# noway/nzcp-circom

Hardware: AMD Instinct MI355X
Metric: groth16_proofs_per_sec_nzcp_live (higher is better)
Workload: dtype u32x8 (256-bit Montgomery integers); 1 GPU; nzcp_liveTest.circom = NZCPPubIdentity(1, 355, 0, 4, 2, 4, 6), single proof: nVars=825434, nConstraints=830227, nPublic=513, domain=2^20, nCoefs=4236306; parallelism=1gpu

## Files before the change

### nzcp-circom_amd/csrc/ec29.cuh

```cuda
#pragma once
#include "ec.cuh"
#include "fq29.cuh"

namespace g16 {

using G1Affine29 = Affine<Fq29Ops>;
using G2Affine29 = Affine<Fq2x29Ops>;
using G1XYZZ29 = XYZZ<Fq29Ops>;
using G2XYZZ29 = XYZZ<Fq2x29Ops>;

template <class F> G16_HD bool x29_is_inf(const XYZZ<F>& p) { return F::is_literal_zero(p.zz); }
template <class F> G16_HD void x29_set_inf(XYZZ<F>& p) {
  p.x = F::zero(); p.y = F::zero(); p.zz = F::zero(); p.zzz = F::zero();
}
template <class F> G16_HD bool x29_diff_is_zero(const typename F::T& d) {
  if (!F::template maybe_zero<7>(d)) return false;
  return F::is_zero(d);
}

template <class F> G16_HD void x29_dbl_affine(XYZZ<F>& r, const Affine<F>& p) {
  using T = typename F::T;
  const T U = F::add(p.y, p.y);
  const T V = F::sqr(U);
  const T W = F::mul(U, V);
// ... 64 lines not shown
    acc.y = F::template sub<2>(F::mul(R, F::template sub<6>(Qv, X3)), F::mul(acc.y, PPP));
  }
  acc.x = X3;
  acc.zz = F::mul(acc.zz, PP);
  acc.zzz = F::mul(acc.zzz, PPP);
  return suspicious;
}

template <class F> G16_HD void x29_add(XYZZ<F>& acc, const XYZZ<F>& q) {
  using T = typename F::T;
  if (x29_is_inf(q)) return;
  if (x29_is_inf(acc)) { acc = q; return; }
  const T U1 = F::mul(acc.x, q.zz);
  const T U2 = F::mul(q.x, acc.zz);
  const T S1 = F::mul(acc.y, q.zzz);
  const T S2 = F::mul(q.y, acc.zzz);
  const T P = F::template sub<2>(U2, U1);
  const T R = F::template sub<2>(S2, S1);
  if (x29_diff_is_zero<F>(P)) {
    if (F::is_zero(R)) x29_dbl(acc);
    else x29_set_inf(acc);
    return;
  }
  const T PP = F::sqr(P);
  const T PPP = F::mul(P, PP);
  const T Qv = F::mul(U1, PP);
  const T X3 = F::sub_b_2c(F::sqr(R), PPP, Qv);
  acc.y = F::template sub<2>(F::mul(R, F::template sub<6>(Qv, X3)), F::mul(S1, PPP));
  acc.x = X3;
  acc.zz = F::mul(F::mul(acc.zz, q.zz), PP);
  acc.zzz = F::mul(F::mul(acc.zzz, q.zzz), PPP);
}

template <class F> G16_HD void a29_neg(Affine<F>& p) { p.y = F::template neg<2>(p.y); }

struct alignas(16) F29Packed { uint32_t v[8]; };
G16_HD F29Packed f29_pack(const F29& a) {
  F29Packed r;
#pragma unroll
  for (int w = 0; w < 8; w++) {
    const int bit = 32 * w, i = bit / 29, o = bit % 29;
    uint64_t x = a.l[i] >> o;
    int have = 29 - o;
    if (i + 1 < 9) { x |= (uint64_t)a.l[i + 1] << have; have += 29; }
    if (have < 32 && i + 2 < 9) x |= (uint64_t)a.l[i + 2] << have;
    r.v[w] = (uint32_t)x;
  }
  return r;
}
G16_HD F29 f29_unpack(const F29Packed& p) {
  F29 t;
#pragma unroll
  for (int i = 0; i < 9; i++) {
    const int bit = 29 * i, w = bit >> 5, o = bit & 31;
    uint64_t x = p.v[w];
    if (w + 1 < 8) x |= (uint64_t)p.v[w + 1] << 32;
    t.l[i] = (uint32_t)(x >> o) & (i < 8 ? kM29 : 0xffffffffu);
  }
  t.pad_ = 0;
  return t;
}
template <class F> struct PackedAffine;
template <> struct alignas(64) PackedAffine<Fq29Ops> { F29Packed x, y; };
template <> struct alignas(64) PackedAffine<Fq2x29Ops> { F29Packed xa, xb, ya, yb; };
G16_HD void a29_pack(PackedAffine<Fq29Ops>& r, const Affine<Fq29Ops>& p) { r.x = f29_pack(p.x); r.y = f29_pack(p.y); }
G16_HD void a29_unpack(Affine<Fq29Ops>& r, const PackedAffine<Fq29Ops>& p) { r.x = f29_unpack(p.x); r.y = f29_unpack(p.y); }
// ... 18 lines not shown
```

### nzcp-circom_amd/csrc/msm.cuh

```cuda
#pragma once
#include <stdlib.h>

#include <atomic>

#include "ec29.cuh"
#include "internal.h"

namespace g16 {

struct MsmPlan {
  uint32_t nsec, n;
  uint32_t sec_begin[kMsmMaxSections];
  int c, Ws;
  uint32_t W, pf, B, low_bits, bins, rps, rows, ones;
  uint32_t salt_bits;
  uint32_t dup_rows, dup_bits;
  uint32_t wb, wx;
  uint32_t wkb;
};
__host__ __device__ __forceinline__ uint32_t msm_win_off(const MsmPlan& pl, uint32_t j) { return j * pl.wb + (j < pl.wx ? j : pl.wx); }
__host__ __device__ __forceinline__ uint32_t msm_win_bits(const MsmPlan& pl, uint32_t j) { return pl.wb + (j < pl.wx ? 1u : 0u); }

__host__ __device__ __forceinline__ uint32_t msm_dup_hash(const uint32_t x[8], uint32_t bits) {
  uint64_t h = 0x9E3779B97F4A7C15ull;
// ... 15 lines not shown
  uint64_t max_tasks = 0;
  uint32_t task_len = 0;
  uint32_t task_len_min = 0;
  uint32_t* h_stat = nullptr;
  uint32_t seg_len = 0;
  uint32_t seg_len_lat = 0, seg_len_thr = 0;
  uint32_t row_pts = 0;
  uint32_t* d_off = nullptr;
  uint32_t* d_toff = nullptr;
  uint32_t* d_foff = nullptr;
  uint32_t* d_tile_a = nullptr;
  uint32_t* d_tile_b = nullptr;
  uint32_t* d_tile_c = nullptr;
  uint2* d_task_desc = nullptr;
  uint4* d_qdesc = nullptr;
  uint32_t* d_class = nullptr;
  uint32_t* d_queue = nullptr;
  uint32_t* d_redo = nullptr;
  void* d_partial = nullptr;
  void* d_bsum = nullptr;
  uint32_t* d_heavy = nullptr;
  uint32_t* d_medium = nullptr;
  uint32_t max_heavy = 0;
  void* d_seg = nullptr;
  void* d_red = nullptr;
  bool reduce_scan = false;
  void* d_canon = nullptr;
  void* d_dseg = nullptr;
  void* d_dred = nullptr;
  hipStream_t st_dup = nullptr;
  hipEvent_t ev_dup_fork = nullptr, ev_dup_join = nullptr;
  uint32_t* d_dcount = nullptr;
  uint32_t* d_dlist = nullptr;
  uint32_t nsec_lane = 0;
  uint8_t* h_pinned = nullptr;
  bool rows_mapped = false;
  size_t out_bytes = 0;
  hipEvent_t ev0 = nullptr, ev1 = nullptr;
  hipEvent_t ev_done = nullptr;
  hipEvent_t trace_ev[4] = {};
  float last_accum_ms = 0.f;
  hipEvent_t gate = nullptr;
  uint32_t waves_per_simd = 0;
  uint32_t chunk_quota = 0;
};

struct MsmWorkspace {
  uint32_t* d_hist = nullptr;
  uint32_t* d_bin_cnt = nullptr;
  uint32_t* d_bin_start = nullptr;
  uint2* d_tmp = nullptr;
  uint32_t* d_sorted = nullptr;
  uint32_t* d_cnt = nullptr;
  uint32_t nb = 0;
  uint32_t* d_dup_cnt = nullptr;
  uint32_t* d_dup_rep = nullptr;
  uint32_t* d_dup_mixed = nullptr;
  const Fr* d_scalars = nullptr;
  bool direct = false;
  uint32_t bin_cap = 0;
  uint32_t dup_chunk = 16, dup_bit_rows = 16;
  uint32_t* h_over = nullptr;
  hipStream_t st_last = nullptr, st2_last = nullptr;
  MsmLaneWs lane[2];
  hipEvent_t ev_sorted = nullptr;
  hipEvent_t trace_ev[4] = {};
  bool launched = false;
  bool empty = false;
};

struct U256 { uint32_t v[8]; };

inline uint32_t msm_seg_len_cfg(int which) {
  struct Cfg { uint32_t v[3]; };
  static const Cfg cfg = [] {
    Cfg c{{8u, 4u, 8u}};
    if (const char* e = getenv("G16_SEG_LEN")) {
      int a = 0, b = 0, d = 0;
      const int k = sscanf(e, "%d,%d,%d", &a, &b, &d);
      if (k >= 1 && a > 0) c.v[0] = (uint32_t)a;
      if (k >= 2 && b > 0) c.v[1] = (uint32_t)b;
      if (k >= 3 && d > 0) c.v[2] = (uint32_t)d;
    }
    for (auto& x : c.v) x = x > 64 ? 64 : x;
    return c;
  }();
  return cfg.v[which];
}

static constexpr uint32_t kTailThreads = 256;
static constexpr uint32_t kRemClasses = 32;
static constexpr uint32_t kTaskChunk = 64;
static constexpr uint32_t kLightTasks = 3;
static constexpr uint32_t kMediumTasks = 64;

struct MsmSmallInit { uint32_t *h_stat, *d_class, *d_queue, *d_heavy, *d_medium; };
int msm_front_end(const MsmGroup& g, MsmWorkspace* ws, const Fr* d_scalars, hipStream_t st);
int msm_build_queue(const MsmGroup& g, MsmWorkspace* ws, MsmLaneWs& ln, hipStream_t st);
int msm_launch_lane_g2(const MsmGroup& g, MsmWorkspace* ws, MsmLaneWs& ln, hipStream_t st);
int msm_convert_bases_g2(const void* in, void* out, uint32_t n);
int msm_precompute_g2(const void* in, void* out, uint32_t n, int ndbl);

template <class F>
__global__ __launch_bounds__(64, F::kAccumWavesPerSimd) void msm_accumulate_kernel(const PackedAffine<F>* __restrict__ bases,
                                                            const uint32_t* __restrict__ sorted,
                                                            const uint32_t* __restrict__ toff, uint32_t nbk,
                                                            uint32_t point_base,
                                                            const uint4* __restrict__ qdesc,
                                                            uint32_t* __restrict__ queue,
                                                            uint32_t* __restrict__ redo,
                                                            XYZZ<F>* __restrict__ partial, uint32_t chunk_quota) {
  const uint32_t total = toff[nbk];
  uint32_t pulled = 0;
  const uint32_t lane = threadIdx.x;
  const unsigned long long lt_mask = (1ull << lane) - 1;
  constexpr uint32_t kNone = 0xffffffffu;
  uint32_t next = 0, chunk_end = 0;
  bool exhausted = false;
  uint32_t my_task = kNone, pending = kNone, cur = 0, end = 0;
  bool bad = false;
  uint4 desc = make_uint4(0, 0, 0, 0);
  XYZZ<F> acc;
  x29_set_inf(acc);
  for (;;) {
    if (my_task != kNone && cur == end) {
      partial[my_task] = acc;
      if (bad) redo[atomicAdd(&queue[1], 1u)] = my_task;
      my_task = kNone;
    }
// ... 461 lines not shown
      if (k == 0 && live) {
        x29_to_canon<F, typename F::CanonOps>(r, v);
        o[0] = r;
      }
    } else {
      for (int d = (int)kPairGroup >> 1; d >= 1; d >>= 1) x29_tree_step<F, (int)kPairGroup>(y, d, k);
      if (k == 0 && live) {
        x29_to_canon<F, typename F::CanonOps>(r, y);
        o[1] = r;
        x29_to_canon<F, typename F::CanonOps>(r, t);
        o[2] = r;
      }
    }
  }
}

static __global__ __launch_bounds__(256) void msm_dup_compact_kernel(const uint32_t* __restrict__ toff, uint32_t B, uint32_t rps,
                                                              uint32_t dup_row0, uint32_t dup_bits, uint32_t sec0,
                                                              uint32_t nsec_lane, const uint32_t* __restrict__ dup_cnt,
                                                              const uint32_t* __restrict__ dup_mixed,
                                                              uint32_t* __restrict__ dcount, uint32_t* __restrict__ dlist) {
  __builtin_amdgcn_s_setprio(3);
  const uint32_t i = blockIdx.x * blockDim.x + threadIdx.x;
  if (i >= (nsec_lane << dup_bits)) return;
  const uint32_t sl = i >> dup_bits, hb = i & ((1u << dup_bits) - 1);
  const size_t di = ((size_t)(sec0 + sl) << dup_bits) + hb;
  if (dup_cnt[di] < kDupMin || dup_mixed[di]) return;
  const uint32_t key = (sl * rps + dup_row0) * B + hb;
  if (toff[key + 1] == toff[key]) return;
  const uint32_t k = atomicAdd(&dcount[sl], 1u);
  dlist[((size_t)sl << dup_bits) + k] = hb;
}

template <class F>
__global__ __launch_bounds__(kTailThreads) void msm_dup_bits_kernel(const XYZZ<F>* __restrict__ partial,
                                                              const XYZZ<F>* __restrict__ bsum,
                                                              const uint32_t* __restrict__ toff, uint32_t B,
                                                              uint32_t rps, uint32_t dup_row0, uint32_t dup_bits,
                                                              uint32_t sec0, uint32_t nsec_lane, uint32_t nchunk,
                                                              uint32_t chunk_bits, uint32_t bit_rows,
                                                              const uint32_t* __restrict__ dcount,
                                                              const uint32_t* __restrict__ dlist,
                                                              const uint32_t* __restrict__ dup_rep,
                                                              const Fr* __restrict__ scalars,
                                                              const uint32_t* __restrict__ src,
                                                              XYZZ<F>* __restrict__ dseg) {
  __builtin_amdgcn_s_setprio(3);
  const uint32_t wid = blockIdx.x * (blockDim.x >> 6) + (threadIdx.x >> 6), lane = threadIdx.x & 63u;
  const uint32_t nrow = nsec_lane * bit_rows;
  if (wid >= nrow * nchunk) return;
  const uint32_t chunk = wid / nrow, row = wid % nrow, bit = row % bit_rows, sl = row / bit_rows;
  const uint32_t wave = row * nchunk + chunk;
  const uint32_t count = dcount[sl], k = chunk * 64 + lane;
  XYZZ<F> acc;
  x29_set_inf(acc);
  if (chunk * 64 < count) {
    if (k < count) {
      const uint32_t hb = dlist[((size_t)sl << dup_bits) + k];
      const Fr v = scalars[src[dup_rep[((size_t)(sec0 + sl) << dup_bits) + hb]]];
      const uint32_t pos = bit * chunk_bits;
      uint64_t w2 = v.v[pos >> 5];
      if ((pos >> 5) + 1 < 8) w2 |= (uint64_t)v.v[(pos >> 5) + 1] << 32;
      const uint32_t cv = (uint32_t)(w2 >> (pos & 31)) & ((1u << chunk_bits) - 1u);
      if (cv) {
        const XYZZ<F> t = msm_bucket_value<F>(partial, bsum, toff, (sl * rps + dup_row0) * B + hb);
        msm_mul_small(acc, t, cv);
      }
    }
    for (int d = 32; d >= 1; d >>= 1) x29_tree_step<F>(acc, d, lane);
  }
  if (lane == 0) dseg[wave] = acc;
}

template <class F>
__global__ __launch_bounds__(kTailThreads) void msm_wave_reduce_kernel(const XYZZ<F>* __restrict__ in, uint32_t nin,
                                                             XYZZ<F>* __restrict__ out, uint32_t nout) {
  __builtin_amdgcn_s_setprio(3);
  const uint32_t j = blockIdx.y, blk = blockIdx.x * (blockDim.x >> 6) + (threadIdx.x >> 6), lane = threadIdx.x & 63u;
  if (blk >= nout) return;
  const uint32_t i = blk * 64 + lane;
  XYZZ<F> p;
  if (i < nin) p = in[(size_t)j * nin + i];
  else x29_set_inf(p);
  for (int d = 32; d >= 1; d >>= 1) x29_tree_step<F>(p, d, lane);
  if (lane == 0) out[(size_t)j * nout + blk] = p;
}

template <class F>
__global__ __launch_bounds__(256) void msm_convert_bases_kernel(const Affine<typename F::CanonOps>* __restrict__ in,
                                                                PackedAffine<F>* __restrict__ out, uint32_t n) {
  const uint32_t i = blockIdx.x * blockDim.x + threadIdx.x;
  if (i >= n) return;
  Affine<F> r;
  a29_from_canon<F, typename F::CanonOps>(r, in[i]);
  PackedAffine<F> pk;
  a29_pack(pk, r);
  out[i] = pk;
}
template <class FC>
__global__ __launch_bounds__(256) void msm_precompute_kernel(const Affine<FC>* __restrict__ in,
                                                             Affine<FC>* __restrict__ out, uint32_t n, int ndbl) {
  const uint32_t i = blockIdx.x * blockDim.x + threadIdx.x;
// ... 115 lines not shown
  uint32_t quota = 0xffffffffu;
  if (ln.chunk_quota) {
    quota = ln.chunk_quota;
    waves = (max_chunks + quota - 1) / quota + 64;
  }
  if (waves > max_chunks) waves = max_chunks;
  if (waves == 0) waves = 1;
  if (ln.gate) G16_HIP(hipStreamWaitEvent(st, ln.gate, 0));
  G16_HIP(hipEventRecord(ln.ev0, st));
  msm_accumulate_kernel<F><<<(unsigned)waves, 64, 0, st>>>((const PackedAffine<F>*)d_bases, ws->d_sorted, ln.d_toff, nbk,
                                                            ln.point_base, ln.d_qdesc, ln.d_queue, ln.d_redo,
                                                            (PT*)ln.d_partial, quota);
  G16_HIP(hipEventRecord(ln.ev1, st));
  msm_redo_kernel<F><<<64, 64, 0, st>>>((const PackedAffine<F>*)d_bases, ws->d_sorted, ln.point_base, ln.d_task_desc,
                                        ln.d_queue, ln.d_redo, (PT*)ln.d_partial);
  msm_combine_light_kernel<FT><<<(nbk + kTailThreads - 1) / kTailThreads, kTailThreads, 0, st>>>((const TPT*)ln.d_partial, ln.d_toff, nbk,
                                                              (TPT*)ln.d_bsum, ln.d_heavy, ln.max_heavy, ln.d_medium,
                                                              msm_light_max(ln), ln.h_stat);
  msm_combine_medium_kernel<FT><<<1024, kTailThreads, 0, st>>>((const TPT*)ln.d_partial, ln.d_toff, (TPT*)ln.d_bsum, ln.d_medium,
                                                              ln.max_heavy);
  msm_combine_heavy_kernel<FT><<<2048, kTailThreads, 0, st>>>((const TPT*)ln.d_partial, ln.d_toff, (TPT*)ln.d_bsum,
                                                   ln.d_heavy, ln.max_heavy);
  mark(1);
  uint32_t nout_pts = ln.row_pts;
  if (g.dup_rows) {
    hipStream_t sd = ln.st_dup ? ln.st_dup : st;
    if (sd != st) {
      G16_HIP(hipEventRecord(ln.ev_dup_fork, st));
      G16_HIP(hipStreamWaitEvent(sd, ln.ev_dup_fork, 0));
    }
    const uint32_t nchunk = (1u << g.dup_bits) >> 6, drows = ln.nsec_lane * ws->dup_bit_rows;
    const uint32_t waves_d = drows * nchunk;
    const uint32_t sec0 = ln.key_lo / (g.rps * g.B), dup_row0 = (uint32_t)g.W + (g.ones ? 1u : 0u);
    G16_HIP(hipMemsetAsync(ln.d_dcount, 0, 16, sd));
    msm_dup_compact_kernel<<<((ln.nsec_lane << g.dup_bits) + 255) / 256, 256, 0, sd>>>(
        ln.d_toff, g.B, g.rps, dup_row0, g.dup_bits, sec0, ln.nsec_lane, ws->d_dup_cnt, ws->d_dup_mixed, ln.d_dcount, ln.d_dlist);
    msm_dup_bits_kernel<FT><<<(waves_d + 3) / 4, kTailThreads, 0, sd>>>(
        (const TPT*)ln.d_partial, (const TPT*)ln.d_bsum, ln.d_toff, g.B, g.rps, dup_row0, g.dup_bits, sec0, ln.nsec_lane, nchunk,
        ws->dup_chunk, ws->dup_bit_rows, ln.d_dcount, ln.d_dlist, ws->d_dup_rep, ws->d_scalars, g.d_src, (TPT*)ln.d_dseg);
    TPT* dcur = (TPT*)ln.d_dseg;
    uint32_t dcnt = nchunk;
    TPT* dbufs[2] = {(TPT*)ln.d_dred, (TPT*)ln.d_dred + (size_t)drows * ((nchunk + 63) / 64)};
    int dflip = 0;
    while (dcnt > 1) {
      const uint32_t nout = (dcnt + 63) / 64;
      msm_wave_reduce_kernel<FT><<<dim3((nout + 3) / 4, drows), kTailThreads, 0, sd>>>(dcur, dcnt, dbufs[dflip], nout);
      dcur = dbufs[dflip];
      dflip ^= 1;
      dcnt = nout;
    }
    msm_to_canon_kernel<F><<<(drows + 63) / 64, 64, 0, sd>>>((const PT*)dcur, (CPT*)ln.d_canon + ln.row_pts, drows);
    G16_HIP(hipGetLastError());
    nout_pts += drows;
    if (sd != st) G16_HIP(hipEventRecord(ln.ev_dup_join, sd));
  }
  if (ln.reduce_scan) {
    const MsmReducePlan rp = msm_reduce_plan(g, ln);
    msm_bucket_reduce_kernel<FT><<<ln.rows * rp.nwg, rp.wg, 0, st>>>((const TPT*)ln.d_partial, (const TPT*)ln.d_bsum, ln.d_toff, rp,
                                                                     (TPT*)ln.d_seg, (CPT*)ln.d_canon);
    mark(2);
    if (rp.nwg > 1) {
      const uint32_t ngroups = (rp.nwg + kPairGroup - 1) / kPairGroup, gpw = 64u / kPairGroup;
      if (ngroups == 1)
        msm_pairs_fold_kernel<FT, true><<<(ln.rows + gpw - 1) / gpw, 64, 0, st>>>((const TPT*)ln.d_seg, rp, 1u, (CPT*)ln.d_canon);
      else
        msm_pairs_fold_kernel<FT, false><<<2 * ((ln.rows * ngroups + gpw - 1) / gpw), 64, 0, st>>>((const TPT*)ln.d_seg, rp, ngroups,
                                                                                            (CPT*)ln.d_canon);
    }
  } else {
    const uint32_t seg_len = ln.seg_len;
    const uint32_t nseg = (g.B + seg_len - 1) / seg_len;
    const uint32_t wave_tree = (nseg % kTailThreads == 0) ? 2u : ((nseg % 64 == 0) ? 1u : 0u);
// ... 32 lines not shown
```

### nzcp-circom_amd/csrc/msm_g1.hip

```cpp
#include <string.h>

#include "msm.cuh"

namespace g16 {

size_t msm_point_bytes(int curve) { return curve == 2 ? sizeof(G2XYZZ) : sizeof(G1XYZZ); }

__device__ __forceinline__ uint32_t msm_extract(const uint32_t s[8], int pos, int c) {
  const int word = pos >> 5, off = pos & 31;
  if (word >= 8) return 0;
  uint64_t v = s[word];
  if (word + 1 < 8) v |= (uint64_t)s[word + 1] << 32;
  return (uint32_t)(v >> off) & ((1u << c) - 1);
}

__device__ __forceinline__ bool msm_load_scalar(const Fr* __restrict__ scalars, const uint32_t* __restrict__ src,
                                                uint32_t g, const U256& K, uint32_t s[8], uint32_t* bits = nullptr) {
  const Fr x = scalars[src ? src[g] : g];
  uint32_t hi = 0;
#pragma unroll
  for (int k = 1; k < 8; k++) hi |= x.v[k];
  const bool one = (hi == 0 && x.v[0] == 1);
  if (bits) {
    uint32_t b = 0;
// ... 349 lines not shown
  __builtin_amdgcn_s_setprio(3);
  __shared__ uint32_t sh_a[256], sh_b[256], sh_c[256];
  const uint32_t tid = threadIdx.x, base = blockIdx.x * kScanTile + tid * 8;
  uint32_t sa = 0, sb = 0, sc = 0;
#pragma unroll
  for (int k = 0; k < 8; k++) {
    const uint32_t v = (base + k < nb) ? cnt[base + k] : 0u;
    sa += v;
    sb += (v + tl - 1) / tl;
    sc += v / tl;
  }
  sh_a[tid] = sa; sh_b[tid] = sb; sh_c[tid] = sc;
  __syncthreads();
  for (uint32_t d = 128; d > 0; d >>= 1) {
    if (tid < d) { sh_a[tid] += sh_a[tid + d]; sh_b[tid] += sh_b[tid + d]; sh_c[tid] += sh_c[tid + d]; }
    __syncthreads();
  }
  if (tid == 0) { tile_a[blockIdx.x] = sh_a[0]; tile_b[blockIdx.x] = sh_b[0]; tile_c[blockIdx.x] = sh_c[0]; }
}

static __global__ __launch_bounds__(1024) void msm_scan_top_kernel(uint32_t* __restrict__ tile_a,
                                                            uint32_t* __restrict__ tile_b,
                                                            uint32_t* __restrict__ tile_c, uint32_t ntiles,
                                                            const uint32_t* __restrict__ off_base,
                                                            uint32_t* __restrict__ total_a,
                                                            uint32_t* __restrict__ total_b,
                                                            uint32_t* __restrict__ total_c, uint32_t max_tasks,
                                                            MsmSmallInit init) {
  __builtin_amdgcn_s_setprio(3);
  __shared__ uint32_t sh_a[1024], sh_b[1024], sh_c[1024];
  const uint32_t tid = threadIdx.x;
  if (tid < 2 * kRemClasses) init.d_class[tid] = 0;
  if (tid < 2) init.d_queue[tid] = 0;
  if (tid == 0) { init.d_heavy[0] = 0; init.d_medium[0] = 0; init.h_stat[3] = 0; }
  const uint32_t chunk = (ntiles + 1023) / 1024;
  const uint32_t lo = tid * chunk, hi = (lo + chunk < ntiles) ? lo + chunk : ntiles;
  uint32_t sa = 0, sb = 0, sc = 0;
  for (uint32_t k = lo; k < hi; k++) { sa += tile_a[k]; sb += tile_b[k]; sc += tile_c[k]; }
  sh_a[tid] = sa; sh_b[tid] = sb; sh_c[tid] = sc;
  __syncthreads();
  for (uint32_t d = 1; d < 1024; d <<= 1) {
    uint32_t va = 0, vb = 0, vc = 0;
    if (tid >= d) { va = sh_a[tid - d]; vb = sh_b[tid - d]; vc = sh_c[tid - d]; }
    __syncthreads();
    sh_a[tid] += va; sh_b[tid] += vb; sh_c[tid] += vc;
    __syncthreads();
  }
  uint32_t pa = sh_a[tid] - sa, pb = sh_b[tid] - sb, pc = sh_c[tid] - sc;
  for (uint32_t k = lo; k < hi; k++) {
    const uint32_t va = tile_a[k], vb = tile_b[k], vc = tile_c[k];
    tile_a[k] = pa; tile_b[k] = pb; tile_c[k] = pc;
    pa += va; pb += vb; pc += vc;
  }
  if (tid == 1023) {
    const uint32_t over = sh_b[1023] > max_tasks ? 1u : 0u;
    init.d_queue[2] = over;
    init.h_stat[2] = over ? sh_b[1023] : 0u;
    *total_a = *off_base + sh_a[1023];
    *total_b = over ? 0u : sh_b[1023];
    *total_c = over ? 0u : sh_c[1023];
    init.h_stat[0] = *off_base + sh_a[1023];
    init.h_stat[1] = *off_base;
  }
}

static __global__ __launch_bounds__(256) void msm_scan_apply_kernel(const uint32_t* __restrict__ cnt, uint32_t nb,
// ... 410 lines not shown
  ln.seg_len_lat = ln.seg_len_thr = ln.seg_len;
  if (ln.reduce_scan && g.dense && !getenv("G16_SEG_LEN")) {
    uint32_t t = ln.seg_len * 2;
    if (g.salt_bits)
      while (t > ln.seg_len && (t > (1u << g.salt_bits) || ((1u << g.salt_bits) % t) != 0)) t >>= 1;
    if (t * 64u <= g.B) ln.seg_len_thr = t;
  }
  const MsmReducePlan rp = msm_reduce_plan(g, ln);
  if (ln.reduce_scan) {
    G16_HIP(hipMalloc(&ln.d_seg, 2 * (size_t)ln.rows * rp.nwg * pb + 256));
  } else {
    const uint64_t nseg = (g.B + ln.seg_len - 1) / ln.seg_len;
    G16_HIP(hipMalloc(&ln.d_seg, (size_t)ln.rows * nseg * pb + 256));
    G16_HIP(hipMalloc(&ln.d_red, 2 * (size_t)ln.rows * ((nseg + 63) / 64) * pb + 256));
  }
  ln.nsec_lane = ln.rows / g.rps;
  ln.row_pts = ln.reduce_scan ? ln.rows * msm_row_out_points(rp) : ln.rows;
  size_t out_pts = ln.row_pts;
  if (g.dup_rows) {
    const size_t nchunk = ((size_t)1 << g.dup_bits) >> 6, drows = (size_t)ln.nsec_lane * g.dup_rows_cap;
    out_pts += drows;
    G16_HIP(hipMalloc(&ln.d_dseg, drows * nchunk * pb + 256));
    G16_HIP(hipMalloc(&ln.d_dred, 2 * drows * ((nchunk + 63) / 64) * pb + 256));
    G16_HIP(hipMalloc(&ln.d_dcount, 64));
    if (curve == 2) {
      int plo = 0, phi = 0;
      G16_HIP(hipDeviceGetStreamPriorityRange(&plo, &phi));
      if (t_aux_prio != kMsmPrioHighest) phi = t_aux_prio;
      G16_HIP(hipStreamCreateWithPriority(&ln.st_dup, hipStreamNonBlocking, phi));
    }
    G16_HIP(hipEventCreateWithFlags(&ln.ev_dup_fork, hipEventDisableTiming));
    G16_HIP(hipEventCreateWithFlags(&ln.ev_dup_join, hipEventDisableTiming));
    G16_HIP(hipMalloc(&ln.d_dlist, ((size_t)ln.nsec_lane << g.dup_bits) * 4 + 64));
  }
  ln.out_bytes = out_pts * cpb;
  G16_HIP(hipHostMalloc((void**)&ln.h_pinned, ln.out_bytes + 256));
  ln.rows_mapped = !(getenv("G16_ROWS_COPY") && atoi(getenv("G16_ROWS_COPY")));
  if (ln.rows_mapped) G16_HIP(hipHostGetDevicePointer(&ln.d_canon, ln.h_pinned, 0));
  else G16_HIP(hipMalloc(&ln.d_canon, ln.out_bytes + 256));
  G16_HIP(hipEventCreate(&ln.ev0));
  G16_HIP(hipEventCreate(&ln.ev1));
  G16_HIP(hipEventCreate(&ln.ev_done));
  return G16_OK;
}

static void lane_destroy(MsmLaneWs& ln) {
  void* ptrs[] = {ln.d_task_desc, ln.d_qdesc, ln.d_class, ln.d_queue, ln.d_redo, ln.d_partial, ln.d_bsum, ln.d_heavy, ln.d_medium,
                  ln.d_seg, ln.d_red, ln.rows_mapped ? nullptr : ln.d_canon, ln.d_off, ln.d_toff, ln.d_foff, ln.d_tile_a, ln.d_tile_b, ln.d_tile_c,
                  ln.d_dseg, ln.d_dred, ln.d_dcount, ln.d_dlist};
  for (void* p : ptrs)
    if (p) (void)hipFree(p);
  if (ln.h_pinned) (void)hipHostFree(ln.h_pinned);
  if (ln.h_stat) (void)hipHostFree(ln.h_stat);
  if (ln.st_dup) (void)hipStreamDestroy(ln.st_dup);
  hipEvent_t evs[] = {ln.ev0, ln.ev1, ln.ev_done, ln.trace_ev[0], ln.trace_ev[1], ln.trace_ev[2], ln.trace_ev[3],
                      ln.ev_dup_fork, ln.ev_dup_join};
  for (hipEvent_t e : evs)
    if (e) (void)hipEventDestroy(e);
  ln = MsmLaneWs();
}

int msm_workspace_create(MsmWorkspace** out, const MsmGroup& g) {
  MsmWorkspace* ws = new MsmWorkspace();
  *out = ws;
  if (g.n == 0) return G16_OK;
  msm_set_throughput(ws, g, false);
  const uint32_t nrb = g.rows * g.bins;
  ws->nb = g.rows * g.B;
  G16_HIP(hipMalloc(&ws->d_hist, ((size_t)g.chunks * nrb + 4) * 4));
  G16_HIP(hipMalloc(&ws->d_bin_cnt, ((size_t)nrb + 4) * 4));
  G16_HIP(hipMalloc(&ws->d_bin_start, ((size_t)nrb + 4) * 4));
  {
    const bool off = getenv("G16_NO_DIRECT_BIN") && atoi(getenv("G16_NO_DIRECT_BIN"));
    uint64_t cap = (g.max_entries * 5 / 2) / nrb + 1024;
    if (const char* e = getenv("G16_TEST_BIN_CAP"))
      if (atoll(e) > 0) cap = (uint64_t)atoll(e);
    ws->direct = g.dense && g.nsec == 1 && !g.ones && !g.dup_rows && !off && cap * nrb < 0x7fffffffull;
    ws->bin_cap = ws->direct ? (uint32_t)cap : 0u;
  }
  G16_HIP(hipHostMalloc((void**)&ws->h_over, 64));
  ws->h_over[0] = 0;
  uint64_t tmp_entries = g.max_entries;
// ... 69 lines not shown
    msm_bin_sort_kernel<<<nrb, 256, 0, st>>>(ws->d_tmp, ws->d_bin_start, pl, ws->d_bin_cnt, ws->bin_cap, ws->h_over, ws->d_cnt,
                                             ws->d_sorted);
    mark(3);
  } else {
    msm_bin_pass_kernel<0><<<g.chunks, kBinThreads, lds, st>>>(d_scalars, g.d_src, pl, K, g.per, g.chunks, ws->d_hist, nullptr,
                                                               ws->d_dup_cnt, ws->d_dup_mixed, nullptr);
    mark(0);
    msm_bin_chunkscan_kernel<<<nrb, 64, 0, st>>>(ws->d_hist, g.chunks, ws->d_bin_cnt);
    msm_bin_scan_kernel<<<1, 1024, 0, st>>>(ws->d_bin_cnt, nrb, ws->d_bin_start, 0xffffffffu);
    mark(1);
    msm_bin_pass_kernel<1><<<g.chunks, kBinThreads, lds, st>>>(d_scalars, g.d_src, pl, K, g.per, g.chunks, ws->d_hist,
                                                               ws->d_bin_start, ws->d_dup_cnt, ws->d_dup_mixed, ws->d_tmp);
    mark(2);
    msm_bin_sort_kernel<<<nrb, 256, 0, st>>>(ws->d_tmp, ws->d_bin_start, pl, nullptr, 0u, nullptr, ws->d_cnt, ws->d_sorted);
    mark(3);
  }
  G16_HIP(hipGetLastError());
  G16_HIP(hipEventRecord(ws->ev_sorted, st));
  return G16_OK;
}

int msm_build_queue(const MsmGroup& g, MsmWorkspace* ws, MsmLaneWs& ln, hipStream_t st) {
  const uint32_t nbk = ln.key_hi - ln.key_lo;
  const uint32_t* cnt = ws->d_cnt + ln.key_lo;
  const uint32_t* off_base = ws->d_bin_start + (size_t)(ln.key_lo / g.B) * g.bins;
  const uint32_t ntiles = (nbk + kScanTile - 1) / kScanTile;
  if (!g.task_len_forced && ln.h_stat[0] > ln.h_stat[1]) {
    const uint64_t e = ln.h_stat[0] - ln.h_stat[1];
    ln.task_len = msm_task_len_for(e / (ln.curve == 2 ? 131072u : 262144u), ln.task_len_min);
  }
  msm_scan_tiles_kernel<<<ntiles, 256, 0, st>>>(cnt, nbk, ln.task_len, ln.d_tile_a, ln.d_tile_b, ln.d_tile_c);
  msm_scan_top_kernel<<<1, 1024, 0, st>>>(ln.d_tile_a, ln.d_tile_b, ln.d_tile_c, ntiles, off_base, ln.d_off + nbk,
                                          ln.d_toff + nbk, ln.d_foff + nbk, (uint32_t)ln.max_tasks,
                                          MsmSmallInit{ln.h_stat, ln.d_class, ln.d_queue, ln.d_heavy, ln.d_medium});
  msm_scan_apply_kernel<<<ntiles, 256, 0, st>>>(cnt, nbk, ln.task_len, ln.d_tile_a, ln.d_tile_b, ln.d_tile_c, off_base,
                                                ln.d_queue, ln.d_off, ln.d_toff, ln.d_foff, ln.d_class);
  msm_task_fill_kernel<<<(nbk + 255) / 256, 256, 0, st>>>(ln.d_off, ln.d_toff, ln.d_foff, nbk, ln.task_len, ln.d_task_desc,
                                                          ln.d_qdesc, ln.d_class, ln.d_class + kRemClasses,
                                                          (uint32_t)ln.max_tasks);
  G16_HIP(hipGetLastError());
  return G16_OK;
}

int msm_launch_front(const MsmGroup& g, MsmWorkspace* ws, const Fr* d_scalars, hipStream_t st) {
  ws->launched = true;
  ws->st_last = st;
  ws->st2_last = nullptr;
  ws->empty = (g.n == 0);
  for (auto& ln : ws->lane) ln.last_accum_ms = 0.f;
  if (g.n == 0) return G16_OK;
  return msm_front_end(g, ws, d_scalars, st);
}

int msm_launch_lanes(const MsmGroup& g, MsmWorkspace* ws, hipStream_t st, hipStream_t st2, hipEvent_t gate1,
                     hipEvent_t gate2) {
  if (g.n == 0) return G16_OK;
  int rc;
  ws->st2_last = st2;
  if (ws->lane[1].active) {
    hipStream_t s2 = st2 ? st2 : st;
    if (s2 != st) G16_HIP(hipStreamWaitEvent(s2, ws->ev_sorted, 0));
    ws->lane[1].gate = gate2;
    if ((rc = msm_launch_lane_g2(g, ws, ws->lane[1], s2))) return rc;
  }
  if (ws->lane[0].active) {
    ws->lane[0].gate = gate1;
    rc = msm_launch_lane_t<Fq29Ops>(g, ws, ws->lane[0], g.d_bases, st);
// ... 10 lines not shown

hipEvent_t msm_event(MsmWorkspace* ws, int which) {
  switch (which) {
    case 0: return ws->ev_sorted;
    case 1: return ws->lane[0].ev0;
    case 2: return ws->lane[0].ev1;
    case 3: return ws->lane[0].active ? ws->lane[0].ev_done : nullptr;
    default: return ws->lane[1].active ? ws->lane[1].ev_done : nullptr;
  }
}

int msm_collect(const MsmGroup& g, MsmWorkspace* ws, MsmResult* out, const std::function<void(const MsmResult&)>* after_g1) {
  for (auto& p : out->g1) xyzz_set_inf(p);
  xyzz_set_inf(out->g2);
  if (!ws->launched || ws->empty) return G16_OK;
  bool overflow = false;
  for (int l = 0; l < 2; l++) {
    MsmLaneWs& ln = ws->lane[l];
    if (!ln.active) continue;
    G16_HIP(hipEventSynchronize(ln.ev_done));
    static const bool trace = getenv("G16_TRACE_HOST") != nullptr;
    if (trace) fprintf(stderr, "[g16 tail] %s lane %d: host saw its row sums at %.3f ms\n", g.dup_rows ? "W" : "H", l, trace_ms());
    (void)hipEventElapsedTime(&ln.last_accum_ms, ln.ev0, ln.ev1);
    if (ln.h_stat[2] || ln.h_stat[3]) {
      set_error(ln.h_stat[2] ? "msm: lane " + std::to_string(l) + " needed " + std::to_string(ln.h_stat[2]) +
                                   " bucket tasks, its buffers hold " + std::to_string(ln.max_tasks)
                             : "msm: lane " + std::to_string(l) + " overflowed its heavy-bucket list");
      overflow = true;
      continue;
    }
    if (g.dup_rows && getenv("G16_DEBUG_DUP")) {
      uint32_t dc[4] = {0, 0, 0, 0};
      (void)hipMemcpy(dc, ln.d_dcount, 16, hipMemcpyDeviceToHost);
      fprintf(stderr, "[g16 dup] lane %d: repeated-value buckets per section: %u %u %u\n", l, dc[0], dc[1], dc[2]);
    }
    const MsmReducePlan rp = msm_reduce_plan(g, ln);
    const uint32_t ngroups = (rp.nwg + kPairGroup - 1) / kPairGroup;
    if (l == 0) {
      const G1XYZZ* rows = reinterpret_cast<const G1XYZZ*>(ln.h_pinned);
      std::vector<G1XYZZ> folded;
      if (ln.reduce_scan && rp.nwg > kPairGroup) {
        folded.resize(ln.rows);
        for (uint32_t r = 0; r < ln.rows; r++)
          msm_fold_row<FqOps>(folded[r], rows + (size_t)r * ngroups * 3, ngroups, rp, msm_row_kind(rp, r));
      }
      const G1XYZZ* rsum = !folded.empty() ? folded.data() : rows;
      const bool merged = g.dup_rows && ws->dup_chunk == (uint32_t)g.c && ws->dup_bit_rows == (uint32_t)g.W;
      std::vector<G1XYZZ> wrow;
      for (int s = 0; s < g.nsec; s++) {
        const G1XYZZ* rs = rsum + (size_t)s * g.rps;
        const G1XYZZ* dup = rows + ln.row_pts + (size_t)s * ws->dup_bit_rows;
        if (merged) {
          wrow.assign(rs, rs + g.W + (g.ones ? 1 : 0));
          for (int j = 0; j < g.W; j++) xyzz_add(wrow[j], dup[j]);
          rs = wrow.data();
        }
        msm_combine_windows<FqOps>(out->g1[s], rs, g.W, g.c, g.ones);
        if (g.dup_rows && !merged) msm_add_bit_sums<FqOps>(out->g1[s], dup, ws->dup_chunk, ws->dup_bit_rows);
      }
      if (after_g1 && *after_g1) (*after_g1)(*out);
    } else {
      const G2XYZZ* rows = reinterpret_cast<const G2XYZZ*>(ln.h_pinned);
      std::vector<G2XYZZ> folded;
      if (ln.reduce_scan && rp.nwg > kPairGroup) {
        folded.resize(ln.rows);
        for (uint32_t r = 0; r < ln.rows; r++)
          msm_fold_row<Fq2Ops>(folded[r], rows + (size_t)r * ngroups * 3, ngroups, rp, msm_row_kind(rp, r));
      }
      const G2XYZZ* rsum = !folded.empty() ? folded.data() : rows;
      const bool merged = g.dup_rows && ws->dup_chunk == (uint32_t)g.c && ws->dup_bit_rows == (uint32_t)g.W;
      std::vector<G2XYZZ> wrow;
      if (merged) {
        wrow.assign(rsum, rsum + g.W + (g.ones ? 1 : 0));
        for (int j = 0; j < g.W; j++) xyzz_add(wrow[j], rows[ln.row_pts + j]);
        rsum = wrow.data();
      }
      msm_combine_windows<Fq2Ops>(out->g2, rsum, g.W, g.c, g.ones);
      if (g.dup_rows && !merged) msm_add_bit_sums<Fq2Ops>(out->g2, rows + ln.row_pts, ws->dup_chunk, ws->dup_bit_rows);
    }
  }
  if (overflow) return G16_E_STATE;
  if (ws->direct && ws->h_over[0]) {
    ws->direct = false;
    ws->h_over[0] = 0;
    int rc = msm_launch_front(g, ws, ws->d_scalars, ws->st_last);
    if (!rc) rc = msm_launch_lanes(g, ws, ws->st_last, ws->st2_last, nullptr, nullptr);
    if (rc) return rc;
    return msm_collect(g, ws, out, after_g1);
  }
  return G16_OK;
}

float msm_last_accum_ms(const MsmWorkspace* ws, int lane) { return ws->lane[lane & 1].last_accum_ms; }
void msm_set_throughput(MsmWorkspace* ws, const MsmGroup& g, bool on) {
  if (!ws) return;
  ws->dup_chunk = on ? g.dup_chunk_wide : g.dup_chunk;
  ws->dup_bit_rows = (254 + ws->dup_chunk - 1) / ws->dup_chunk;
  for (auto& ln : ws->lane)
    if (ln.active) ln.seg_len = on ? ln.seg_len_thr : ln.seg_len_lat;
}
void msm_set_waves(MsmWorkspace* ws, uint32_t waves_g1, uint32_t waves_g2) {
  ws->lane[0].waves_per_simd = waves_g1;
  ws->lane[1].waves_per_simd = waves_g2;
}
void msm_set_quota(MsmWorkspace* ws, uint32_t quota_g1, uint32_t quota_g2) {
  ws->lane[0].chunk_quota = quota_g1;
  ws->lane[1].chunk_quota = quota_g2;
}
float msm_event_offset_ms(MsmWorkspace* ws, hipEvent_t base, int lane, int which) {
  float t = 0.f;
  const MsmLaneWs& ln = ws->lane[lane & 1];
  hipEvent_t e = which < 4 ? ws->trace_ev[which] : which == 4 ? ln.ev0 : which == 5 ? ln.ev1 : ln.trace_ev[(which - 6) & 3];
  if (e && hipEventQuery(e) == hipSuccess) (void)hipEventElapsedTime(&t, base, e);
  return t;
}

}
```

Baseline: 282.6 proofs/s.

## Precompute per-position multiple tables for repeated-value buckets in dup-bit MSM

Adds a table kernel that, for each repeated-value bucket, precomputes multiples 1..15 of the bucket point shifted by each 4-bit sub-position of the chunk. The dup-bits kernel then sums table lookups instead of running a double-and-add scalar multiply for every bit row. This removes redundant small-scalar multiplications repeated across rows, at the cost of a large extra device buffer, an extra launch, and XYZZ table reads. It also folds the dcount memset into the scan-top init kernel, saving one async memset. The table path is enabled only in throughput mode.

```diff
diff --git a/nzcp-circom_amd/csrc/ec29.cuh b/nzcp-circom_amd/csrc/ec29.cuh
--- a/nzcp-circom_amd/csrc/ec29.cuh
+++ b/nzcp-circom_amd/csrc/ec29.cuh
@@ -120,6 +120,55 @@
   acc.zzz = F::mul(F::mul(acc.zzz, q.zzz), PPP);
 }
 
+static constexpr uint32_t kDupSubBits = 4;
+static constexpr uint32_t kDupTabMul = (1u << kDupSubBits) - 1;
+static constexpr uint32_t kDupTabPosMax = 4;
+G16_HD uint32_t x29_dup_positions(uint32_t chunk_bits) { return (chunk_bits + kDupSubBits - 1) / kDupSubBits; }
+G16_HD uint32_t x29_dup_pos_max(uint32_t chunk_bits, uint32_t p) {
+  const uint32_t w = chunk_bits - kDupSubBits * p;
+  return w >= kDupSubBits ? kDupTabMul : (1u << w) - 1u;
+}
+static constexpr uint32_t kDupSplitPos = 3;
+template <class F> G16_HD void x29_dup_table_range(XYZZ<F>* tab, const XYZZ<F>& t, uint32_t p, uint32_t jlo, uint32_t jhi) {
+  const uint32_t nbase = kDupSubBits * p;
+  const uint32_t nd = nbase + (jlo == 1 ? (jhi >= 2 ? 1u : 0u) : 3u);
+  XYZZ<F> cur = t, b = t;
+  for (uint32_t i = 0; i < nd; i++) {
+    x29_dbl(cur);
+    if (i + 1 == nbase) b = cur;
+  }
+  uint32_t j = 9;
+  if (jlo == 1) {
+    tab[0] = b;
+    if (jhi < 2) return;
+    tab[1] = cur;
+    j = 3;
+  }
+  for (; j <= jhi; j++) {
+    x29_add(cur, b);
+    tab[j - 1] = cur;
+  }
+}
+G16_HD bool x29_dup_table_half_range(uint32_t p, uint32_t half, uint32_t jmax, uint32_t& jlo, uint32_t& jhi) {
+  const bool split = p >= kDupSplitPos && jmax > 8u;
+  jlo = half ? 9u : 1u;
+  jhi = (half || !split) ? jmax : 8u;
+  return half == 0 || split;
+}
+template <class F> G16_HD void x29_dup_chunk_entry(XYZZ<F>& q, const XYZZ<F>* tab, uint32_t cv, uint32_t p) {
+  const uint32_t d = (cv >> (kDupSubBits * p)) & kDupTabMul;
+  if (d) q = tab[p * kDupTabMul + d - 1];
+  else x29_set_inf(q);
+}
+template <class F> G16_HD void x29_dup_chunk_sum(XYZZ<F>& acc, const XYZZ<F>* tab, uint32_t cv, uint32_t npos) {
+  x29_set_inf(acc);
+  for (uint32_t p = 0; p < npos; p++) {
+    XYZZ<F> e;
+    x29_dup_chunk_entry(e, tab, cv, p);
+    x29_add(acc, e);
+  }
+}
+
 template <class F> G16_HD void a29_neg(Affine<F>& p) { p.y = F::template neg<2>(p.y); }
 
 struct alignas(16) F29Packed { uint32_t v[8]; };
diff --git a/nzcp-circom_amd/csrc/msm.cuh b/nzcp-circom_amd/csrc/msm.cuh
--- a/nzcp-circom_amd/csrc/msm.cuh
+++ b/nzcp-circom_amd/csrc/msm.cuh
@@ -71,6 +71,8 @@
   hipEvent_t ev_dup_fork = nullptr, ev_dup_join = nullptr;
   uint32_t* d_dcount = nullptr;
   uint32_t* d_dlist = nullptr;
+  void* d_dtab = nullptr;
+  size_t dtab_bytes = 0;
   uint32_t nsec_lane = 0;
   uint8_t* h_pinned = nullptr;
   bool rows_mapped = false;
@@ -99,6 +101,7 @@
   bool direct = false;
   uint32_t bin_cap = 0;
   uint32_t dup_chunk = 16, dup_bit_rows = 16;
+  bool dup_tables = false;
   uint32_t* h_over = nullptr;
   hipStream_t st_last = nullptr, st2_last = nullptr;
   MsmLaneWs lane[2];
@@ -133,7 +136,8 @@
 static constexpr uint32_t kLightTasks = 3;
 static constexpr uint32_t kMediumTasks = 64;
 
-struct MsmSmallInit { uint32_t *h_stat, *d_class, *d_queue, *d_heavy, *d_medium; };
+struct MsmSmallInit { uint32_t *h_stat, *d_class, *d_queue, *d_heavy, *d_medium, *d_dcount; };
+static constexpr uint32_t kDupTabCap = 1024;
 int msm_front_end(const MsmGroup& g, MsmWorkspace* ws, const Fr* d_scalars, hipStream_t st);
 int msm_build_queue(const MsmGroup& g, MsmWorkspace* ws, MsmLaneWs& ln, hipStream_t st);
 int msm_launch_lane_g2(const MsmGroup& g, MsmWorkspace* ws, MsmLaneWs& ln, hipStream_t st);
@@ -661,7 +665,49 @@
   dlist[((size_t)sl << dup_bits) + k] = hb;
 }
 
-template <class F>
+__host__ __device__ __forceinline__ uint32_t msm_dup_chunk_value(const uint32_t v[8], uint32_t row, uint32_t chunk_bits) {
+  const uint32_t pos = row * chunk_bits;
+  uint64_t w2 = v[pos >> 5];
+  if ((pos >> 5) + 1 < 8) w2 |= (uint64_t)v[(pos >> 5) + 1] << 32;
+  return (uint32_t)(w2 >> (pos & 31)) & ((1u << chunk_bits) - 1u);
+}
+
+template <class F>
+__global__ __launch_bounds__(kTailThreads) void msm_dup_table_kernel(const XYZZ<F>* __restrict__ partial,
+                                                               const XYZZ<F>* __restrict__ bsum,
+                                                               const uint32_t* __restrict__ toff, uint32_t B,
+                                                               uint32_t rps, uint32_t dup_row0, uint32_t dup_bits,
+                                                               uint32_t sec0, uint32_t nsec_lane, uint32_t nchunk_tab,
+                                                               uint32_t chunk_bits, uint32_t bit_rows,
+                                                               const uint32_t* __restrict__ dcount,
+                                                               const uint32_t* __restrict__ dlist,
+                                                               const uint32_t* __restrict__ dup_rep,
+                                                               const Fr* __restrict__ scalars,
+                                                               const uint32_t* __restrict__ src,
+                                                               XYZZ<F>* __restrict__ tab) {
+  __builtin_amdgcn_s_setprio(3);
+  const uint32_t wid = blockIdx.x * (blockDim.x >> 6) + (threadIdx.x >> 6), lane = threadIdx.x & 63u;
+  const uint32_t npos = x29_dup_positions(chunk_bits), nrow = nsec_lane * npos * 2u;
+  if (wid >= nrow * nchunk_tab) return;
+  const uint32_t chunk = wid / nrow, r = wid % nrow, half = r & 1u, p = (r >> 1) % npos, sl = (r >> 1) / npos;
+  uint32_t count = dcount[sl];
+  if (count > kDupTabCap) count = kDupTabCap;
+  const uint32_t k = chunk * 64 + lane, jmax = x29_dup_pos_max(chunk_bits, p);
+  uint32_t jlo, jhi;
+  if (k >= count || !x29_dup_table_half_range(p, half, jmax, jlo, jhi)) return;
+  const uint32_t hb = dlist[((size_t)sl << dup_bits) + k];
+  const Fr v = scalars[src[dup_rep[((size_t)(sec0 + sl) << dup_bits) + hb]]];
+  bool need = false;
+  for (uint32_t row = 0; row < bit_rows; row++) {
+    const uint32_t d = (msm_dup_chunk_value(v.v, row, chunk_bits) >> (kDupSubBits * p)) & kDupTabMul;
+    need |= d >= jlo && d <= jhi;
+  }
+  if (!need) return;
+  const XYZZ<F> t = msm_bucket_value<F>(partial, bsum, toff, (sl * rps + dup_row0) * B + hb);
+  x29_dup_table_range(tab + (((size_t)sl * kDupTabCap + k) * npos + p) * kDupTabMul, t, p, jlo, jhi);
+}
+
+template <class F, bool TAB>
 __global__ __launch_bounds__(kTailThreads) void msm_dup_bits_kernel(const XYZZ<F>* __restrict__ partial,
                                                               const XYZZ<F>* __restrict__ bsum,
                                                               const uint32_t* __restrict__ toff, uint32_t B,
@@ -673,6 +719,7 @@
                                                               const uint32_t* __restrict__ dup_rep,
                                                               const Fr* __restrict__ scalars,
                                                               const uint32_t* __restrict__ src,
+                                                              const XYZZ<F>* __restrict__ tab,
                                                               XYZZ<F>* __restrict__ dseg) {
   __builtin_amdgcn_s_setprio(3);
   const uint32_t wid = blockIdx.x * (blockDim.x >> 6) + (threadIdx.x >> 6), lane = threadIdx.x & 63u;
@@ -683,20 +730,46 @@
   const uint32_t count = dcount[sl], k = chunk * 64 + lane;
   XYZZ<F> acc;
   x29_set_inf(acc);
-  if (chunk * 64 < count) {
+  if (!TAB) {
+    if (chunk * 64 < count) {
+      if (k < count) {
+        const uint32_t hb = dlist[((size_t)sl << dup_bits) + k];
+        const Fr v = scalars[src[dup_rep[((size_t)(sec0 + sl) << dup_bits) + hb]]];
+        const uint32_t cv = msm_dup_chunk_value(v.v, bit, chunk_bits);
+        if (cv) {
+          const XYZZ<F> t = msm_bucket_value<F>(partial, bsum, toff, (sl * rps + dup_row0) * B + hb);
+          msm_mul_small(acc, t, cv);
+        }
+      }
+      for (int d = 32; d >= 1; d >>= 1) x29_tree_step<F>(acc, d, lane);
+    }
+  } else if (chunk * 64 < count) {
+    const bool tabbed = chunk * 64 < kDupTabCap;
+    const uint32_t npos = x29_dup_positions(chunk_bits);
+    const XYZZ<F>* mine = tab + ((size_t)sl * kDupTabCap + (tabbed ? k : 0u)) * npos * kDupTabMul;
+    uint32_t cv = 0;
     if (k < count) {
       const uint32_t hb = dlist[((size_t)sl << dup_bits) + k];
       const Fr v = scalars[src[dup_rep[((size_t)(sec0 + sl) << dup_bits) + hb]]];
-      const uint32_t pos = bit * chunk_bits;
-      uint64_t w2 = v.v[pos >> 5];
-      if ((pos >> 5) + 1 < 8) w2 |= (uint64_t)v.v[(pos >> 5) + 1] << 32;
-      const uint32_t cv = (uint32_t)(w2 >> (pos & 31)) & ((1u << chunk_bits) - 1u);
-      if (cv) {
+      cv = msm_dup_chunk_value(v.v, bit, chunk_bits);
+      if (cv && !tabbed) {
         const XYZZ<F> t = msm_bucket_value<F>(partial, bsum, toff, (sl * rps + dup_row0) * B + hb);
         msm_mul_small(acc, t, cv);
-      }
-    }
-    for (int d = 32; d >= 1; d >>= 1) x29_tree_step<F>(acc, d, lane);
+        cv = 0;
+      }
+    }
+#pragma unroll 1
+    for (uint32_t step = 0; step < npos + 6u; step++) {
+      XYZZ<F> q;
+      if (step < npos) {
+        x29_dup_chunk_entry(q, mine, cv, step);
+      } else {
+        const int d = 32 >> (step - npos);
+        q = xyzz_shfl_down<F>(acc, d);
+        if (lane >= (uint32_t)d) x29_set_inf(q);
+      }
+      x29_add(acc, q);
+    }
   }
   if (lane == 0) dseg[wave] = acc;
 }
@@ -878,12 +951,24 @@
     const uint32_t nchunk = (1u << g.dup_bits) >> 6, drows = ln.nsec_lane * ws->dup_bit_rows;
     const uint32_t waves_d = drows * nchunk;
     const uint32_t sec0 = ln.key_lo / (g.rps * g.B), dup_row0 = (uint32_t)g.W + (g.ones ? 1u : 0u);
-    G16_HIP(hipMemsetAsync(ln.d_dcount, 0, 16, sd));
     msm_dup_compact_kernel<<<((ln.nsec_lane << g.dup_bits) + 255) / 256, 256, 0, sd>>>(
         ln.d_toff, g.B, g.rps, dup_row0, g.dup_bits, sec0, ln.nsec_lane, ws->d_dup_cnt, ws->d_dup_mixed, ln.d_dcount, ln.d_dlist);
-    msm_dup_bits_kernel<FT><<<(waves_d + 3) / 4, kTailThreads, 0, sd>>>(
-        (const TPT*)ln.d_partial, (const TPT*)ln.d_bsum, ln.d_toff, g.B, g.rps, dup_row0, g.dup_bits, sec0, ln.nsec_lane, nchunk,
-        ws->dup_chunk, ws->dup_bit_rows, ln.d_dcount, ln.d_dlist, ws->d_dup_rep, ws->d_scalars, g.d_src, (TPT*)ln.d_dseg);
+    if (ws->dup_tables) {
+      const uint32_t nchunk_tab = nchunk < kDupTabCap / 64u ? nchunk : kDupTabCap / 64u;
+      const uint32_t waves_t = ln.nsec_lane * x29_dup_positions(ws->dup_chunk) * 2u * nchunk_tab;
+      msm_dup_table_kernel<FT><<<(waves_t + 3) / 4, kTailThreads, 0, sd>>>(
+          (const TPT*)ln.d_partial, (const TPT*)ln.d_bsum, ln.d_toff, g.B, g.rps, dup_row0, g.dup_bits, sec0, ln.nsec_lane, nchunk_tab,
+          ws->dup_chunk, ws->dup_bit_rows, ln.d_dcount, ln.d_dlist, ws->d_dup_rep, ws->d_scalars, g.d_src, (TPT*)ln.d_dtab);
+      msm_dup_bits_kernel<FT, true><<<(waves_d + 3) / 4, kTailThreads, 0, sd>>>(
+          (const TPT*)ln.d_partial, (const TPT*)ln.d_bsum, ln.d_toff, g.B, g.rps, dup_row0, g.dup_bits, sec0, ln.nsec_lane, nchunk,
+          ws->dup_chunk, ws->dup_bit_rows, ln.d_dcount, ln.d_dlist, ws->d_dup_rep, ws->d_scalars, g.d_src, (const TPT*)ln.d_dtab,
+          (TPT*)ln.d_dseg);
+    } else {
+      msm_dup_bits_kernel<FT, false><<<(waves_d + 3) / 4, kTailThreads, 0, sd>>>(
+          (const TPT*)ln.d_partial, (const TPT*)ln.d_bsum, ln.d_toff, g.B, g.rps, dup_row0, g.dup_bits, sec0, ln.nsec_lane, nchunk,
+          ws->dup_chunk, ws->dup_bit_rows, ln.d_dcount, ln.d_dlist, ws->d_dup_rep, ws->d_scalars, g.d_src, (const TPT*)ln.d_dtab,
+          (TPT*)ln.d_dseg);
+    }
     TPT* dcur = (TPT*)ln.d_dseg;
     uint32_t dcnt = nchunk;
     TPT* dbufs[2] = {(TPT*)ln.d_dred, (TPT*)ln.d_dred + (size_t)drows * ((nchunk + 63) / 64)};
diff --git a/nzcp-circom_amd/csrc/msm_g1.hip b/nzcp-circom_amd/csrc/msm_g1.hip
--- a/nzcp-circom_amd/csrc/msm_g1.hip
+++ b/nzcp-circom_amd/csrc/msm_g1.hip
@@ -405,6 +405,7 @@
   const uint32_t tid = threadIdx.x;
   if (tid < 2 * kRemClasses) init.d_class[tid] = 0;
   if (tid < 2) init.d_queue[tid] = 0;
+  if (init.d_dcount && tid < 4) init.d_dcount[tid] = 0;
   if (tid == 0) { init.d_heavy[0] = 0; init.d_medium[0] = 0; init.h_stat[3] = 0; }
   const uint32_t chunk = (ntiles + 1023) / 1024;
   const uint32_t lo = tid * chunk, hi = (lo + chunk < ntiles) ? lo + chunk : ntiles;
@@ -881,6 +882,8 @@
     G16_HIP(hipEventCreateWithFlags(&ln.ev_dup_fork, hipEventDisableTiming));
     G16_HIP(hipEventCreateWithFlags(&ln.ev_dup_join, hipEventDisableTiming));
     G16_HIP(hipMalloc(&ln.d_dlist, ((size_t)ln.nsec_lane << g.dup_bits) * 4 + 64));
+    ln.dtab_bytes = (size_t)ln.nsec_lane * kDupTabCap * kDupTabPosMax * kDupTabMul * pb;
+    G16_HIP(hipMalloc(&ln.d_dtab, ln.dtab_bytes + 256));
   }
   ln.out_bytes = out_pts * cpb;
   G16_HIP(hipHostMalloc((void**)&ln.h_pinned, ln.out_bytes + 256));
@@ -896,7 +899,7 @@
 static void lane_destroy(MsmLaneWs& ln) {
   void* ptrs[] = {ln.d_task_desc, ln.d_qdesc, ln.d_class, ln.d_queue, ln.d_redo, ln.d_partial, ln.d_bsum, ln.d_heavy, ln.d_medium,
                   ln.d_seg, ln.d_red, ln.rows_mapped ? nullptr : ln.d_canon, ln.d_off, ln.d_toff, ln.d_foff, ln.d_tile_a, ln.d_tile_b, ln.d_tile_c,
-                  ln.d_dseg, ln.d_dred, ln.d_dcount, ln.d_dlist};
+                  ln.d_dseg, ln.d_dred, ln.d_dcount, ln.d_dlist, ln.d_dtab};
   for (void* p : ptrs)
     if (p) (void)hipFree(p);
   if (ln.h_pinned) (void)hipHostFree(ln.h_pinned);
@@ -1032,7 +1035,7 @@
   msm_scan_tiles_kernel<<<ntiles, 256, 0, st>>>(cnt, nbk, ln.task_len, ln.d_tile_a, ln.d_tile_b, ln.d_tile_c);
   msm_scan_top_kernel<<<1, 1024, 0, st>>>(ln.d_tile_a, ln.d_tile_b, ln.d_tile_c, ntiles, off_base, ln.d_off + nbk,
                                           ln.d_toff + nbk, ln.d_foff + nbk, (uint32_t)ln.max_tasks,
-                                          MsmSmallInit{ln.h_stat, ln.d_class, ln.d_queue, ln.d_heavy, ln.d_medium});
+                                          MsmSmallInit{ln.h_stat, ln.d_class, ln.d_queue, ln.d_heavy, ln.d_medium, ln.d_dcount});
   msm_scan_apply_kernel<<<ntiles, 256, 0, st>>>(cnt, nbk, ln.task_len, ln.d_tile_a, ln.d_tile_b, ln.d_tile_c, off_base,
                                                 ln.d_queue, ln.d_off, ln.d_toff, ln.d_foff, ln.d_class);
   msm_task_fill_kernel<<<(nbk + 255) / 256, 256, 0, st>>>(ln.d_off, ln.d_toff, ln.d_foff, nbk, ln.task_len, ln.d_task_desc,
@@ -1109,7 +1112,8 @@
     if (g.dup_rows && getenv("G16_DEBUG_DUP")) {
       uint32_t dc[4] = {0, 0, 0, 0};
       (void)hipMemcpy(dc, ln.d_dcount, 16, hipMemcpyDeviceToHost);
-      fprintf(stderr, "[g16 dup] lane %d: repeated-value buckets per section: %u %u %u\n", l, dc[0], dc[1], dc[2]);
+      fprintf(stderr, "[g16 dup] lane %d: repeated-value buckets per section: %u %u %u; table of %u per section, %.1f MB\n", l,
+              dc[0], dc[1], dc[2], kDupTabCap, (double)ln.dtab_bytes / 1048576.0);
     }
     const MsmReducePlan rp = msm_reduce_plan(g, ln);
     const uint32_t ngroups = (rp.nwg + kPairGroup - 1) / kPairGroup;
@@ -1173,6 +1177,7 @@
   if (!ws) return;
   ws->dup_chunk = on ? g.dup_chunk_wide : g.dup_chunk;
   ws->dup_bit_rows = (254 + ws->dup_chunk - 1) / ws->dup_chunk;
+  ws->dup_tables = on;
   for (auto& ln : ws->lane)
     if (ln.active) ln.seg_len = on ? ln.seg_len_thr : ln.seg_len_lat;
 }
```

Result: slower. 278.7 proofs/s (-1.4%).
